# Symb0x76/ChineseChessZero

Measured on NVIDIA B200. Metric: self-play moves/sec at 400 playouts, higher is better.
Workload: dtype bf16

## Files before the change

chinesechesszero_b200/_lib.py:

```python
from __future__ import annotations

import ctypes
import os

import numpy as np
import torch

from . import build as _build

BOARD_BYTES = 96
MAX_MOVES = 128
N_ACTIONS = 2086
PLANE_ELEMS = 10710
KEY_WINDOW = 128

FLAG_CHECK, FLAG_NOMOVES, FLAG_INSUFFICIENT, FLAG_FOURFOLD, FLAG_SIXTY = 1, 2, 4, 8, 16
FLAG_TIE_MASK = FLAG_INSUFFICIENT | FLAG_FOURFOLD | FLAG_SIXTY
STATUS_EXPAND_FAILED, STATUS_TREE_DROPPED = 1, 2
STATUS_NODE_OVERFLOW = STATUS_EXPAND_FAILED
ADVANCE_NEW_GAME, ADVANCE_DROP_TREE, ADVANCE_KEEP = -1, -2, -3
CTL_HEAD, CTL_TAIL, CTL_EXPAND_FAILED, CTL_TREES_DROPPED, CTL_MIN_FREE, CTL_WORDS = 0, 1, 2, 3, 4, 8
NODE_BYTES = 24
MAX_CHILDREN = 119
POLICY_PROBS, POLICY_LOGITS = 0, 1
DEDUP_MAX_BOARDS = 16384
CONV_VARIANT_1CTA, CONV_VARIANT_PAIR, CONV_VARIANT_2PAIRS, CONV_VARIANT_4PAIRS = 1, 2, 2 | 32, 2 | 64

EXPORTS = (
    "ccz_version", "ccz_last_error", "ccz_init", "ccz_action_table", "ccz_set_order_policy", "ccz_get_order_policy",
    "ccz_boards_start",
    "ccz_movegen_encode", "ccz_board_keys_init", "ccz_board_push", "ccz_mcts_pool_init", "ccz_mcts_reset",
    "ccz_mcts_reserve", "ccz_mcts_migrate", "ccz_mcts_select",
    "ccz_mcts_expand_backup", "ccz_mcts_root_visits", "ccz_mcts_advance", "ccz_replay_pack", "ccz_conv3x3_c256", "ccz_conv3x3_plan", "ccz_stem_lookup",
    "ccz_heads_pack", "ccz_conv3x3_c256_count", "ccz_stem_lookup_count", "ccz_heads_pack_rows", "ccz_leaf_unique",
)


class CczError(RuntimeError):
    pass


# ... 334 lines not shown
def conv3x3_c256(x: torch.Tensor, w: torch.Tensor, bias: torch.Tensor, skip: torch.Tensor | None = None,
                 out: torch.Tensor | None = None, variant: int = 0, count: torch.Tensor | None = None) -> torch.Tensor:
    cl = torch.channels_last
    if x.dtype != torch.bfloat16 or w.dtype != torch.bfloat16 or bias.dtype != torch.float32:
        raise CczError("conv3x3_c256: x and w must be bfloat16, bias float32")
    if tuple(x.shape[1:]) != (256, 10, 9) or tuple(w.shape) != (256, 256, 3, 3) or bias.numel() != 256:
        raise CczError("conv3x3_c256: shapes must be x (n,256,10,9), w (256,256,3,3), bias (256,)")
    if not x.is_contiguous(memory_format=cl) or not w.is_contiguous(memory_format=cl):
        raise CczError("conv3x3_c256: x and w must be channels_last")
    if skip is not None and (skip.shape != x.shape or skip.dtype != x.dtype or not skip.is_contiguous(memory_format=cl)):
        raise CczError("conv3x3_c256: skip must match x (bf16, channels_last)")
    if out is None:
        out = torch.empty_like(x, memory_format=cl)
    elif out.shape != x.shape or out.dtype != x.dtype or not out.is_contiguous(memory_format=cl):
        raise CczError("conv3x3_c256: out must match x (bf16, channels_last)")
    if not 0 <= variant < 128:
        raise CczError("conv3x3_c256: variant out of range (see ccz_conv3x3_c256 in include/ccz_b200.h)")
    if not (x.is_cuda and w.is_cuda and bias.is_cuda and out.is_cuda):
        raise CczError("device tensor expected (the C ABI takes device pointers)")
    sk = None if skip is None else skip.data_ptr()
    with torch.cuda.device(x.device):
        if count is None:
            check(load().ccz_conv3x3_c256(x.data_ptr(), w.data_ptr(), bias.data_ptr(), sk, out.data_ptr(), int(x.shape[0]),
                                          int(variant), stream_ptr(x.device)), "ccz_conv3x3_c256")
        else:
            _check_count(count, x.device)
            check(load().ccz_conv3x3_c256_count(x.data_ptr(), w.data_ptr(), bias.data_ptr(), sk, out.data_ptr(), int(x.shape[0]),
                                                count.data_ptr(), int(variant), stream_ptr(x.device)), "ccz_conv3x3_c256_count")
    return out


# ... 60 lines not shown
```

chinesechesszero_b200/csrc/ccz_b200.cu:

```cuda
#include "../../include/ccz_b200.h"

#include <cuda_runtime.h>

#include <cstdio>
#include <cstdlib>
#include <cstring>
#include <utility>
#include <string>

#include "ccz_movegen.cuh"
#include "ccz_mcts.cuh"
#include "ccz_replay.cuh"
#include "ccz_conv.cuh"
#include "ccz_stem.cuh"
#include "ccz_heads.cuh"
#include "ccz_dedup.cuh"

#ifndef CCZ_CONV_DEFAULT_PAIRS
#define CCZ_CONV_DEFAULT_PAIRS 1
#endif

namespace {

thread_local std::string g_err;
// ... 397 lines not shown
    const int threads = 256;
    const long long blocks = (words + threads - 1) / threads;
    if (blocks > 0x7fffffffll) return fail(-1, "ccz_replay_pack: n too large");
    ccz::replay_states_kernel<<<(unsigned)blocks, threads, 0, s>>>(d_hist_boards, d_turn_plane, n,
                                                                   static_cast<uint32_t *>(d_states_f16));
    if (int rc = check_launch("replay_states_kernel")) return rc;
    CCZ_CUDA(cudaMemsetAsync(d_pi, 0, (size_t)2 * n * ccz::N_ACTIONS * sizeof(double), s));
    ccz::replay_pi_kernel<<<(n * 32 + threads - 1) / threads, threads, 0, s>>>(d_acts, d_probs, d_counts, n, d_pi);
    return check_launch("replay_pi_kernel");
}

}

namespace {

int conv3x3_c256_impl(const char *name, const void *d_x, const void *d_w, const float *d_bias, const void *d_skip, void *d_y,
                      int n_boards, const int32_t *d_count, int variant, ccz_stream_t s) {
    namespace cv = ccz::conv;
    std::string e_name(name);
    auto bad = [&](int code, const char *what) { return fail(code, (e_name + ": " + what).c_str()); };
    if (n_boards < 0) return bad(-1, "n_boards < 0");
    if (n_boards == 0) return 0;
    if (!d_x || !d_w || !d_bias || !d_y) return bad(-1, "NULL pointer");
    if (d_y == d_x) return bad(-1, "output must not alias the input (halo reads)");
    if (variant < 0 || variant >= 128) return bad(-1, "bad variant");
    int cta_group = variant & 3;
    const int tail_split = !(variant & 4), dbg = (variant >> 3) & 3;
    int pairs = 1 << ((variant >> 5) & 3);
#ifndef CCZ_CONV_EXPERIMENTS
    if (dbg) return bad(-1, "the load-skipping measurement variants need a -DCCZ_CONV_EXPERIMENTS build");
#endif
    if (variant == 0) { cta_group = 2; pairs = CCZ_CONV_DEFAULT_PAIRS; }
    if (cta_group == 0) cta_group = 2;
    if (cta_group == 3 || pairs > 4 || (cta_group == 1 && pairs != 1))
        return bad(-1, "unsupported variant (cta_group 1|2, pairs 1|2|4, pairs > 1 needs cta_group 2)");
    if (((uintptr_t)d_x | (uintptr_t)d_w | (uintptr_t)d_y | (uintptr_t)d_skip) & 15)
        return bad(-1, "pointers must be 16-byte aligned");
    static cv::Driver drv;
    if (const char *err = cv::driver_init(drv)) return fail(-3, err);
    const long long m = (long long)n_boards * cv::BOARD_HW;
    const int rows_per_tile = cv::BM * cta_group * pairs;
    const int n_tiles = (int)((m + rows_per_tile - 1) / rows_per_tile);
    CUtensorMap tx, tw, ts, ty;
    if (!cv::encode_im2col(drv, &tx, d_x, n_boards)) return bad(-3, "cuTensorMapEncodeIm2col(x) failed");
    if (!cv::encode_rows(drv, &tw, d_w, cv::BN, 9 * cv::C, (uint32_t)(cv::BN / cta_group / pairs)))
        return bad(-3, "cuTensorMapEncodeTiled(w) failed");
    if (!cv::encode_rows(drv, &ty, d_y, (uint64_t)m, cv::C, cv::BM)) return bad(-3, "cuTensorMapEncodeTiled(y) failed");
    if (d_skip) {
        if (!cv::encode_rows(drv, &ts, d_skip, (uint64_t)m, cv::C, cv::BM)) return bad(-3, "cuTensorMapEncodeTiled(skip) failed");
    } else {
        ts = ty;
    }
    cudaError_t e;
#define CCZ_CONV_LAUNCH_C(CG, PAIRS, CNT)                                                                                  \
    (d_skip ? cv::launch_variant<CG, PAIRS, true, CNT>(tx, tw, ts, ty, d_bias, n_tiles, tail_split, dbg, d_count, n_boards, s) \
            : cv::launch_variant<CG, PAIRS, false, CNT>(tx, tw, ts, ty, d_bias, n_tiles, tail_split, dbg, d_count, n_boards, s))
#define CCZ_CONV_LAUNCH(CG, PAIRS) (d_count ? CCZ_CONV_LAUNCH_C(CG, PAIRS, true) : CCZ_CONV_LAUNCH_C(CG, PAIRS, false))
    if (cta_group == 1) e = CCZ_CONV_LAUNCH(1, 1);
    else if (pairs == 1) e = CCZ_CONV_LAUNCH(2, 1);
    else if (pairs == 2) e = CCZ_CONV_LAUNCH(2, 2);
    else e = CCZ_CONV_LAUNCH(2, 4);
#undef CCZ_CONV_LAUNCH
#undef CCZ_CONV_LAUNCH_C
    if (e != cudaSuccess) return fail(-2, "conv3x3_c256_kernel launch", e);
    return 0;
}

int stem_lookup_impl(const char *name, const uint8_t *d_boards, int n, const int32_t *d_count, const void *d_table,
                     const float *d_bias_turn, void *d_y, ccz_stream_t s) {
    namespace st = ccz::stem;
    std::string e_name(name);
    if (n < 0) return fail(-1, (e_name + ": n < 0").c_str());
    if (n == 0) return 0;
    if (!d_boards || !d_table || !d_bias_turn || !d_y) return fail(-1, (e_name + ": NULL pointer").c_str());
    if (((uintptr_t)d_boards & 3) || (((uintptr_t)d_table | (uintptr_t)d_bias_turn | (uintptr_t)d_y) & 15))
        return fail(-1, (e_name + ": pointers must be 16-byte aligned (boards 4-byte)").c_str());
// ... 41 lines not shown
extern "C" {

int ccz_conv3x3_c256(const void *d_x, const void *d_w, const float *d_bias, const void *d_skip, void *d_y, int n_boards,
                     int variant, ccz_stream_t s) {
    return conv3x3_c256_impl("ccz_conv3x3_c256", d_x, d_w, d_bias, d_skip, d_y, n_boards, nullptr, variant, s);
}

int ccz_conv3x3_c256_count(const void *d_x, const void *d_w, const float *d_bias, const void *d_skip, void *d_y, int capacity,
                           const int32_t *d_n_boards, int variant, ccz_stream_t s) {
    if (!d_n_boards) return fail(-1, "ccz_conv3x3_c256_count: d_n_boards is NULL");
    return conv3x3_c256_impl("ccz_conv3x3_c256_count", d_x, d_w, d_bias, d_skip, d_y, capacity, d_n_boards, variant, s);
}

int ccz_conv3x3_plan(int n_boards, int variant, int resident_clusters, int32_t *out) {
    namespace cv = ccz::conv;
    if (n_boards <= 0 || resident_clusters <= 0 || !out || variant < 0 || variant >= 128)
        return fail(-1, "ccz_conv3x3_plan: bad argument");
    int cta_group = variant & 3, pairs = 1 << ((variant >> 5) & 3);
    if (variant == 0) { cta_group = 2; pairs = CCZ_CONV_DEFAULT_PAIRS; }
    if (cta_group == 0) cta_group = 2;
    if (cta_group == 3 || pairs > 4 || (cta_group == 1 && pairs != 1)) return fail(-1, "ccz_conv3x3_plan: unsupported variant");
    const long long m = (long long)n_boards * cv::BOARD_HW;
    const int rows_per_tile = cv::BM * cta_group * pairs;
    const int n_tiles = (int)((m + rows_per_tile - 1) / rows_per_tile);
    const cv::Plan pl = cv::plan_items(n_tiles, resident_clusters, !(variant & 4));
    out[0] = rows_per_tile; out[1] = n_tiles; out[2] = pl.n_items; out[3] = pl.n_full; out[4] = pl.split_log2; out[5] = pl.clusters;
    return 0;
}

int ccz_stem_lookup(const uint8_t *d_boards, int n, const void *d_table, const float *d_bias_turn, void *d_y, ccz_stream_t s) {
    return stem_lookup_impl("ccz_stem_lookup", d_boards, n, nullptr, d_table, d_bias_turn, d_y, s);
}

int ccz_stem_lookup_count(const uint8_t *d_boards, int capacity, const int32_t *d_n_boards, const void *d_table, const float *d_bias_turn,
                          void *d_y, ccz_stream_t s) {
    if (!d_n_boards) return fail(-1, "ccz_stem_lookup_count: d_n_boards is NULL");
    return stem_lookup_impl("ccz_stem_lookup_count", d_boards, capacity, d_n_boards, d_table, d_bias_turn, d_y, s);
}
// ... 36 lines not shown
```

chinesechesszero_b200/csrc/ccz_conv.cuh:

```cuda
#pragma once

#include <cuda.h>
#include <cuda_bf16.h>
#include <cuda_runtime.h>

#include <cstdint>

#ifndef CCZ_CONV_BACKOFF_NS
#define CCZ_CONV_BACKOFF_NS 256
#endif

namespace ccz {
namespace conv {

constexpr int C = 256;
constexpr int BOARD_H = 10, BOARD_W = 9, BOARD_HW = 90;
constexpr int BM = 128;
constexpr int BN = 256;
constexpr int BK = 64;
constexpr int KBLOCKS = 9 * (C / BK);
constexpr int UMMA_K = 16;
constexpr int THREADS = 256;

template <int CG>
struct Cfg {
    static constexpr int B_ROWS = BN / CG;
    static constexpr int A_BYTES = BM * BK * 2;
    static constexpr int B_BYTES = B_ROWS * BK * 2;
    static constexpr int STAGE_BYTES = A_BYTES + B_BYTES;
    static constexpr int STAGES = CG == 2 ? 5 : 3;
    static constexpr int STAGING_BYTES = BM * BN * 2;
    static constexpr int BIAS_BYTES = BN * 4;
    static constexpr int BAR_BYTES = 256;
    static constexpr int SMEM_BYTES = 1024  + STAGES * STAGE_BYTES + STAGING_BYTES + BIAS_BYTES + BAR_BYTES;
};

__device__ __forceinline__ uint32_t smem_u32(const void *p) { return (uint32_t)__cvta_generic_to_shared(p); }

__device__ __forceinline__ uint32_t cluster_ctarank() {
    uint32_t r;
    asm volatile("mov.u32 %0, %%cluster_ctarank;" : "=r"(r));
    return r;
}
__device__ __forceinline__ uint32_t mapa(uint32_t addr, uint32_t rank) {
    uint32_t r;
// ... 172 lines not shown
    asm volatile("barrier.cluster.arrive.release.aligned;\nbarrier.cluster.wait.acquire.aligned;" ::: "memory");
}

__device__ __forceinline__ uint64_t umma_desc_sw128(uint32_t smem_addr) {
    return (uint64_t)((smem_addr >> 4) & 0x3FFF) | (1ull << 16) | (64ull << 32) | (1ull << 46) | (2ull << 61);
}
__host__ __device__ constexpr uint32_t umma_idesc(int m, int n) {
    return (1u << 4) | (1u << 7) | (1u << 10) | ((uint32_t)(n >> 3) << 17) | ((uint32_t)(m >> 4) << 24);
}

__device__ __forceinline__ uint32_t pack_bf16x2(float lo, float hi) {
    __nv_bfloat162 t = __floats2bfloat162_rn(lo, hi);
    return *reinterpret_cast<uint32_t *>(&t);
}

struct WorkItem {
    int tile, n_off, n_w;
};
__device__ __forceinline__ WorkItem work_item(int i, int n_full, int split_log2) {
    if (i < n_full) return {i, 0, BN};
    const int j = i - n_full, n_w = BN >> split_log2;
    return {n_full + (j >> split_log2), (j & ((1 << split_log2) - 1)) * n_w, n_w};
}

struct Plan {
    int n_items, n_full, split_log2, clusters;
};
__host__ __device__ inline Plan plan_items(int n_tiles, int clusters, bool tail_split) {
    const int rem = n_tiles % clusters;
    int split_log2 = 0;
    if (tail_split && rem > 0) {
        while (split_log2 < 2 && (rem << (split_log2 + 1)) <= clusters) ++split_log2;
    }
    Plan p;
    p.split_log2 = split_log2;
    p.n_full = split_log2 ? n_tiles - rem : n_tiles;
    p.n_items = p.n_full + (split_log2 ? rem << split_log2 : 0);
    p.clusters = clusters > p.n_items ? p.n_items : clusters;
    return p;
}

template <int CG, int PAIRS, bool HAS_SKIP, bool DEV_COUNT>
__global__ void __launch_bounds__(THREADS, 1)
conv3x3_c256_kernel(const __grid_constant__ CUtensorMap tm_x, const __grid_constant__ CUtensorMap tm_w,
                    const __grid_constant__ CUtensorMap tm_skip, const __grid_constant__ CUtensorMap tm_y, const float *__restrict__ bias,
                    int n_items, int n_full, int split_log2, int dbg, const int32_t *__restrict__ d_count, int count_cap, int tail_split) {
    using K = Cfg<CG>;
    extern __shared__ uint8_t smem_raw[];
    const uint32_t smem_base = (smem_u32(smem_raw) + 1023u) & ~1023u;
    const uint32_t a_smem = smem_base;
    const uint32_t b_smem = a_smem + K::STAGES * K::A_BYTES;
    const uint32_t staging = b_smem + K::STAGES * K::B_BYTES;
    const uint32_t bias_smem = staging + K::STAGING_BYTES;
    const uint32_t bars = bias_smem + K::BIAS_BYTES;
    const uint32_t bar_full = bars;
    const uint32_t bar_empty = bars + 8 * K::STAGES;
    const uint32_t bar_tfull = bars + 16 * K::STAGES;
    const uint32_t bar_tempty = bar_tfull + 16;
    const uint32_t bar_skip = bar_tempty + 16;
    const uint32_t bar_stfree = bar_skip + 8;
    const uint32_t tmem_slot = bar_stfree + 8;
    uint8_t *const smem_gen = smem_raw + (smem_base - smem_u32(smem_raw));

    const int warp = threadIdx.x >> 5, lane = threadIdx.x & 31;
    static_assert(CG == 2 || PAIRS == 1, "weight multicast needs CTA pairs");
    constexpr int CLUSTER = CG * PAIRS;
    const uint32_t rank = CLUSTER > 1 ? cluster_ctarank() : 0u;
    const uint32_t prank = rank % CG, pair_id = rank / CG, lead_rank = rank - prank;
    const int cluster_id = blockIdx.x / CLUSTER, n_clusters = gridDim.x / CLUSTER;
    if constexpr (DEV_COUNT) {
        const int nb = min(max(*d_count, 0), count_cap), rows_per_tile = BM * CLUSTER;
        const Plan pl = plan_items((nb * BOARD_HW + rows_per_tile - 1) / rows_per_tile, n_clusters, tail_split != 0);
        n_items = pl.n_items;
        n_full = pl.n_full;
        split_log2 = pl.split_log2;
    }

    if (warp == 0 && lane == 0) {
        tma_prefetch_desc(&tm_x);
        tma_prefetch_desc(&tm_w);
        tma_prefetch_desc(&tm_y);
        if (HAS_SKIP) tma_prefetch_desc(&tm_skip);
    }
    if (warp == 1 && lane == 0) {
        for (int i = 0; i < K::STAGES; ++i) {
            mbar_init(bar_full + 8 * i, 1);
            mbar_init(bar_empty + 8 * i, PAIRS);
        }
        for (int i = 0; i < 2; ++i) {
            mbar_init(bar_tfull + 8 * i, 1);
            mbar_init(bar_tempty + 8 * i, 4 * CG);
        }
        mbar_init(bar_skip, 1);
        mbar_init(bar_stfree, 1);
        asm volatile("fence.mbarrier_init.release.cluster;" ::: "memory");
    }
    if (warp == 2) tmem_alloc<CG>(tmem_slot, 512);
    if (warp >= 4) {
        const int t = threadIdx.x - 128;
        reinterpret_cast<float *>(smem_gen + (bias_smem - smem_base))[t] = bias[t];
        reinterpret_cast<float *>(smem_gen + (bias_smem - smem_base))[t + 128] = bias[t + 128];
    }
    tc_fence_before();
    if constexpr (CLUSTER > 1) cluster_sync_all(); else __syncthreads();
    tc_fence_after();
    const uint32_t tmem_base = *reinterpret_cast<volatile uint32_t *>(smem_gen + (tmem_slot - smem_base));

    if (warp == 0) {
        if (lane == 0) {
            const uint32_t full0 = CG == 2 ? mapa(bar_full, lead_rank) : bar_full;
            constexpr int SLICE_ROWS = K::B_ROWS / PAIRS;
            uint16_t mc_mask = 0;
            for (int j = 0; j < PAIRS; ++j) mc_mask |= (uint16_t)(1u << (j * CG + prank));
            int stage = 0;
            uint32_t phase = 0;
            for (int item = cluster_id; item < n_items; item += n_clusters) {
                const WorkItem wi = work_item(item, n_full, split_log2);
                const int m0 = ((wi.tile * PAIRS + (int)pair_id) * CG + (int)prank) * BM;
                const int b_row = wi.n_off + (int)prank * (wi.n_w / CG);
                const int img = m0 / BOARD_HW, rem = m0 - img * BOARD_HW;
                const int p = rem / BOARD_W, q = rem - p * BOARD_W;
                for (int kb = 0; kb < KBLOCKS; ++kb) {
                    const int tap = kb >> 2, c0 = (kb & 3) * BK;
                    const int r = tap / 3, s = tap - 3 * r;
                    mbar_wait(bar_empty + 8 * stage, phase ^ 1);
                    const bool do_a = !((dbg & 2) && (kb & 1)), do_b = !((dbg & 1) && (kb & 1));
                    if (prank == 0) mbar_expect_tx(bar_full + 8 * stage, CG * ((do_a ? K::A_BYTES : 0) + (do_b ? K::B_BYTES : 0)));
                    if (do_a) tma_load_im2col<CG>(a_smem + stage * K::A_BYTES, &tm_x, full0 + 8 * stage, c0, q - 1, p - 1, img, (uint16_t)s, (uint16_t)r);
                    if constexpr (PAIRS == 1) {
                        if (do_b) tma_load_2d<CG>(b_smem + stage * K::B_BYTES, &tm_w, full0 + 8 * stage, kb * BK, b_row);
                    } else {
                        tma_load_2d_mc(b_smem + stage * K::B_BYTES + (int)pair_id * SLICE_ROWS * 128, &tm_w, full0 + 8 * stage, kb * BK,
                                       b_row + (int)pair_id * SLICE_ROWS, mc_mask);
                    }
                    if (++stage == K::STAGES) { stage = 0; phase ^= 1; }
                }
            }
        }
    } else if (warp == 1) {
        if (prank == 0 && lane == 0) {
            constexpr uint16_t mask_cluster = (uint16_t)((1u << CLUSTER) - 1);
            const uint16_t mask_pair = (uint16_t)(((1u << CG) - 1) << lead_rank);
            int stage = 0;
            uint32_t phase = 0, acc = 0, acc_phase = 0;
            for (int item = cluster_id; item < n_items; item += n_clusters) {
                const uint32_t idesc = umma_idesc(BM * CG, work_item(item, n_full, split_log2).n_w);
                mbar_wait_cluster(bar_tempty + 8 * acc, acc_phase ^ 1);
                tc_fence_after();
                const uint32_t d_tmem = tmem_base + acc * BN;
                for (int kb = 0; kb < KBLOCKS; ++kb) {
                    mbar_wait(bar_full + 8 * stage, phase);
                    tc_fence_after();
                    const uint64_t a_desc = umma_desc_sw128(a_smem + stage * K::A_BYTES);
                    const uint64_t b_desc = umma_desc_sw128(b_smem + stage * K::B_BYTES);
#pragma unroll
                    for (int k = 0; k < BK / UMMA_K; ++k)
                        umma_bf16<CG>(d_tmem, a_desc + 2 * k, b_desc + 2 * k, idesc, (uint32_t)((kb | k) != 0));
                    umma_commit<CG>(bar_empty + 8 * stage, mask_cluster);
                    if (++stage == K::STAGES) { stage = 0; phase ^= 1; }
                }
                umma_commit<CG>(bar_tfull + 8 * acc, mask_pair);
                if (++acc == 2) { acc = 0; acc_phase ^= 1; }
            }
        }
    } else if (warp == 3) {
        if (HAS_SKIP && lane == 0) {
            uint32_t it = 0;
            for (int item = cluster_id; item < n_items; item += n_clusters, ++it) {
                const WorkItem wi = work_item(item, n_full, split_log2);
                const int m0 = ((wi.tile * PAIRS + (int)pair_id) * CG + (int)prank) * BM;
                mbar_wait_relaxed(bar_stfree, (it & 1) ^ 1);
                mbar_expect_tx(bar_skip, (wi.n_w / 64) * (BM * 128));
                for (int g = 0; g < wi.n_w / 64; ++g) tma_load_2d<1>(staging + g * (BM * 128), &tm_skip, bar_skip, wi.n_off + g * 64, m0);
            }
        }
    } else if (warp >= 4) {
        const int quarter = warp - 4, row = quarter * 32 + lane;
        const uint32_t tempty0 = CG == 2 ? mapa(bar_tempty, lead_rank) : bar_tempty;
        const float *bias_s = reinterpret_cast<const float *>(smem_gen + (bias_smem - smem_base));
        uint8_t *stg = smem_gen + (staging - smem_base);
        uint32_t acc = 0, acc_phase = 0, it = 0;
        for (int item = cluster_id; item < n_items; item += n_clusters, ++it) {
            const WorkItem wi = work_item(item, n_full, split_log2);
            const int m0 = ((wi.tile * PAIRS + (int)pair_id) * CG + (int)prank) * BM;
            if (HAS_SKIP) mbar_wait_relaxed(bar_skip, it & 1);
            mbar_wait_relaxed(bar_tfull + 8 * acc, acc_phase);
            tc_fence_after();
            const uint32_t t_row = tmem_base + ((uint32_t)(quarter * 32) << 16) + acc * BN;
#pragma unroll 1
            for (int chunk = 0; chunk < wi.n_w / 32; ++chunk) {
                uint32_t v[32];
                tmem_ld32(t_row + chunk * 32, v);
                tmem_ld_wait();
                uint8_t *box_row = stg + (chunk >> 1) * (BM * 128) + row * 128;
#pragma unroll
                for (int j = 0; j < 4; ++j) {
                    const int c16 = (chunk & 1) * 4 + j;
                    uint4 *cell = reinterpret_cast<uint4 *>(box_row + ((c16 ^ (row & 7)) << 4));
                    const float4 b0 = *reinterpret_cast<const float4 *>(bias_s + wi.n_off + chunk * 32 + j * 8);
                    const float4 b1 = *reinterpret_cast<const float4 *>(bias_s + wi.n_off + chunk * 32 + j * 8 + 4);
                    float f[8] = {__uint_as_float(v[j * 8 + 0]) + b0.x, __uint_as_float(v[j * 8 + 1]) + b0.y,
                                  __uint_as_float(v[j * 8 + 2]) + b0.z, __uint_as_float(v[j * 8 + 3]) + b0.w,
                                  __uint_as_float(v[j * 8 + 4]) + b1.x, __uint_as_float(v[j * 8 + 5]) + b1.y,
                                  __uint_as_float(v[j * 8 + 6]) + b1.z, __uint_as_float(v[j * 8 + 7]) + b1.w};
                    if (HAS_SKIP) {
                        const uint4 sk = *cell;
                        const uint32_t w[4] = {sk.x, sk.y, sk.z, sk.w};
#pragma unroll
                        for (int e = 0; e < 4; ++e) {
                            f[2 * e] += __uint_as_float(w[e] << 16);
                            f[2 * e + 1] += __uint_as_float(w[e] & 0xFFFF0000u);
                        }
                    }
                    uint4 o;
                    o.x = pack_bf16x2(fmaxf(f[0], 0.f), fmaxf(f[1], 0.f));
                    o.y = pack_bf16x2(fmaxf(f[2], 0.f), fmaxf(f[3], 0.f));
                    o.z = pack_bf16x2(fmaxf(f[4], 0.f), fmaxf(f[5], 0.f));
                    o.w = pack_bf16x2(fmaxf(f[6], 0.f), fmaxf(f[7], 0.f));
                    *cell = o;
                }
            }
            tc_fence_before();
            __syncwarp();
            if (lane == 0) {
                if constexpr (CG == 2) mbar_arrive_cluster(tempty0 + 8 * acc); else mbar_arrive(bar_tempty + 8 * acc);
            }
            if (++acc == 2) { acc = 0; acc_phase ^= 1; }
            fence_proxy_async();
            asm volatile("bar.sync 1, 128;" ::: "memory");
            if (threadIdx.x == 128) {
                for (int g = 0; g < wi.n_w / 64; ++g) tma_store_2d(&tm_y, staging + g * (BM * 128), wi.n_off + g * 64, m0);
                tma_store_commit();
                tma_store_wait_read();
                if (HAS_SKIP) mbar_arrive(bar_stfree);
            }
            asm volatile("bar.sync 1, 128;" ::: "memory");
        }
        if (threadIdx.x == 128) tma_store_wait_all();
    }

    __syncwarp();
    tc_fence_before();
    if constexpr (CLUSTER > 1) cluster_sync_all(); else __syncthreads();
    if (warp == 2) {
        tc_fence_after();
        tmem_dealloc<CG>(tmem_base, 512);
    }
}

typedef CUresult (*EncodeTiledFn)(CUtensorMap *, CUtensorMapDataType, cuuint32_t, void *, const cuuint64_t *, const cuuint64_t *,
                                  const cuuint32_t *, const cuuint32_t *, CUtensorMapInterleave, CUtensorMapSwizzle, CUtensorMapL2promotion,
// ... 30 lines not shown
    const cuuint32_t es[2] = {1, 1};
    return d.tiled(m, CU_TENSOR_MAP_DATA_TYPE_BFLOAT16, 2, const_cast<void *>(ptr), dims, strides, box, es, CU_TENSOR_MAP_INTERLEAVE_NONE,
                   CU_TENSOR_MAP_SWIZZLE_128B, CU_TENSOR_MAP_L2_PROMOTION_L2_256B, CU_TENSOR_MAP_FLOAT_OOB_FILL_NONE) == CUDA_SUCCESS;
}

inline bool encode_im2col(const Driver &d, CUtensorMap *m, const void *ptr, int n) {
    const cuuint64_t dims[4] = {(cuuint64_t)C, (cuuint64_t)BOARD_W, (cuuint64_t)BOARD_H, (cuuint64_t)n};
    const cuuint64_t strides[3] = {(cuuint64_t)C * 2, (cuuint64_t)C * 2 * BOARD_W, (cuuint64_t)C * 2 * BOARD_HW};
    const int lower[2] = {-1, -1}, upper[2] = {-1, -1};
    const cuuint32_t es[4] = {1, 1, 1, 1};
    return d.im2col(m, CU_TENSOR_MAP_DATA_TYPE_BFLOAT16, 4, const_cast<void *>(ptr), dims, strides, lower, upper, BK, BM, es,
                    CU_TENSOR_MAP_INTERLEAVE_NONE, CU_TENSOR_MAP_SWIZZLE_128B, CU_TENSOR_MAP_L2_PROMOTION_L2_256B,
                    CU_TENSOR_MAP_FLOAT_OOB_FILL_NONE) == CUDA_SUCCESS;
}

template <int CG, int PAIRS, bool HAS_SKIP, bool DEV_COUNT>
inline cudaError_t launch_variant(const CUtensorMap &tx, const CUtensorMap &tw, const CUtensorMap &ts, const CUtensorMap &ty, const float *bias,
                                  int n_tiles, int tail_split, int dbg, const int32_t *d_count, int count_cap, cudaStream_t stream) {
    auto kern = conv3x3_c256_kernel<CG, PAIRS, HAS_SKIP, DEV_COUNT>;
    constexpr int CLUSTER = CG * PAIRS;
    static int max_clusters_dev[64] = {0};
    int dev = 0, n_sm = 0;
    cudaError_t e0 = cudaGetDevice(&dev);
    if (e0 != cudaSuccess) return e0;
    if (dev < 0 || dev >= 64) return cudaErrorInvalidDevice;
    int &max_clusters = max_clusters_dev[dev];
    cudaLaunchConfig_t cfg = {};
    cfg.blockDim = dim3(THREADS);
    cfg.dynamicSmemBytes = Cfg<CG>::SMEM_BYTES;
    cfg.stream = stream;
    cudaLaunchAttribute at[1];
    at[0].id = cudaLaunchAttributeClusterDimension;
    at[0].val.clusterDim.x = CLUSTER;
    at[0].val.clusterDim.y = 1;
    at[0].val.clusterDim.z = 1;
    cfg.attrs = at;
    cfg.numAttrs = 1;
    if (!max_clusters) {
        cudaError_t e = cudaDeviceGetAttribute(&n_sm, cudaDevAttrMultiProcessorCount, dev);
        if (e != cudaSuccess) return e;
        e = cudaFuncSetAttribute(kern, cudaFuncAttributeMaxDynamicSharedMemorySize, Cfg<CG>::SMEM_BYTES);
        if (e != cudaSuccess) return e;
        cfg.gridDim = dim3((unsigned)(n_sm / CLUSTER * CLUSTER));
        int n = 0;
        e = cudaOccupancyMaxActiveClusters(&n, kern, &cfg);
        if (e != cudaSuccess) return e;
        if (n < 1) return cudaErrorInvalidConfiguration;
        max_clusters = n < n_sm / CLUSTER ? n : n_sm / CLUSTER;
    }
    if constexpr (DEV_COUNT) {
        cfg.gridDim = dim3((unsigned)(max_clusters * CLUSTER));
        return cudaLaunchKernelEx(&cfg, kern, tx, tw, ts, ty, bias, 0, 0, 0, dbg, d_count, count_cap, tail_split);
    }
    const Plan pl = plan_items(n_tiles, max_clusters, tail_split != 0);
    cfg.gridDim = dim3((unsigned)(pl.clusters * CLUSTER));
    return cudaLaunchKernelEx(&cfg, kern, tx, tw, ts, ty, bias, pl.n_items, pl.n_full, pl.split_log2, dbg, (const int32_t *)nullptr, 0, 0);
// ... 5 lines not shown
```

Measured before the change: 404.9.

## Add two-M-tile-per-CTA conv variant sharing weight tiles, default for pairs

Adds an MT=2 mode to the 3x3 conv kernel. In this mode each CTA pair computes two 128-row M tiles against one loaded weight (B) stage, which halves B traffic per output row. The mode uses two TMEM accumulators, 8 epilogue warps that split columns, and fewer pipeline stages. It becomes the default when pairs==1, which it is by default. The cost is a larger smem stage, shallower pipelining, more threads, and a more complex MMA and epilogue schedule with new phase-tracking assumptions.

Result: slower. 388.6 (median of 6 runs) (-4.0%).

```diff
diff --git a/chinesechesszero_b200/_lib.py b/chinesechesszero_b200/_lib.py
--- a/chinesechesszero_b200/_lib.py
+++ b/chinesechesszero_b200/_lib.py
@@ -25,6 +25,7 @@
 POLICY_PROBS, POLICY_LOGITS = 0, 1
 DEDUP_MAX_BOARDS = 16384
 CONV_VARIANT_1CTA, CONV_VARIANT_PAIR, CONV_VARIANT_2PAIRS, CONV_VARIANT_4PAIRS = 1, 2, 2 | 32, 2 | 64
+CONV_VARIANT_PAIR_2M = 2 | 128
 
 EXPORTS = (
     "ccz_version", "ccz_last_error", "ccz_init", "ccz_action_table", "ccz_set_order_policy", "ccz_get_order_policy",
@@ -389,7 +390,7 @@
         out = torch.empty_like(x, memory_format=cl)
     elif out.shape != x.shape or out.dtype != x.dtype or not out.is_contiguous(memory_format=cl):
         raise CczError("conv3x3_c256: out must match x (bf16, channels_last)")
-    if not 0 <= variant < 128:
+    if not 0 <= variant < 256:
         raise CczError("conv3x3_c256: variant out of range (see ccz_conv3x3_c256 in include/ccz_b200.h)")
     if not (x.is_cuda and w.is_cuda and bias.is_cuda and out.is_cuda):
         raise CczError("device tensor expected (the C ABI takes device pointers)")
diff --git a/chinesechesszero_b200/csrc/ccz_b200.cu b/chinesechesszero_b200/csrc/ccz_b200.cu
--- a/chinesechesszero_b200/csrc/ccz_b200.cu
+++ b/chinesechesszero_b200/csrc/ccz_b200.cu
@@ -435,6 +435,21 @@
 
 namespace {
 
+struct ConvTiling {
+    int cta_group, pairs, mt;
+};
+const char *conv_tiling(int variant, ConvTiling &t) {
+    if (variant < 0 || variant >= 256) return "bad variant";
+    t.cta_group = variant & 3;
+    t.pairs = 1 << ((variant >> 5) & 3);
+    t.mt = variant & 128 ? 2 : 1;
+    if (variant == 0) { t.cta_group = 2; t.pairs = CCZ_CONV_DEFAULT_PAIRS; t.mt = t.pairs == 1 ? 2 : 1; }
+    if (t.cta_group == 0) t.cta_group = 2;
+    if (t.cta_group == 3 || t.pairs > 4 || (t.cta_group == 1 && t.pairs != 1) || (t.mt == 2 && (t.cta_group != 2 || t.pairs != 1)))
+        return "unsupported variant (cta_group 1|2, pairs 1|2|4, pairs > 1 and two M tiles need cta_group 2, two M tiles need pairs 1)";
+    return nullptr;
+}
+
 int conv3x3_c256_impl(const char *name, const void *d_x, const void *d_w, const float *d_bias, const void *d_skip, void *d_y,
                       int n_boards, const int32_t *d_count, int variant, ccz_stream_t s) {
     namespace cv = ccz::conv;
@@ -444,23 +459,19 @@
     if (n_boards == 0) return 0;
     if (!d_x || !d_w || !d_bias || !d_y) return bad(-1, "NULL pointer");
     if (d_y == d_x) return bad(-1, "output must not alias the input (halo reads)");
-    if (variant < 0 || variant >= 128) return bad(-1, "bad variant");
-    int cta_group = variant & 3;
+    ConvTiling t;
+    if (const char *err = conv_tiling(variant, t)) return bad(-1, err);
+    const int cta_group = t.cta_group, pairs = t.pairs;
     const int tail_split = !(variant & 4), dbg = (variant >> 3) & 3;
-    int pairs = 1 << ((variant >> 5) & 3);
 #ifndef CCZ_CONV_EXPERIMENTS
     if (dbg) return bad(-1, "the load-skipping measurement variants need a -DCCZ_CONV_EXPERIMENTS build");
 #endif
-    if (variant == 0) { cta_group = 2; pairs = CCZ_CONV_DEFAULT_PAIRS; }
-    if (cta_group == 0) cta_group = 2;
-    if (cta_group == 3 || pairs > 4 || (cta_group == 1 && pairs != 1))
-        return bad(-1, "unsupported variant (cta_group 1|2, pairs 1|2|4, pairs > 1 needs cta_group 2)");
     if (((uintptr_t)d_x | (uintptr_t)d_w | (uintptr_t)d_y | (uintptr_t)d_skip) & 15)
         return bad(-1, "pointers must be 16-byte aligned");
     static cv::Driver drv;
     if (const char *err = cv::driver_init(drv)) return fail(-3, err);
     const long long m = (long long)n_boards * cv::BOARD_HW;
-    const int rows_per_tile = cv::BM * cta_group * pairs;
+    const int rows_per_tile = cv::BM * t.mt * cta_group * pairs;
     const int n_tiles = (int)((m + rows_per_tile - 1) / rows_per_tile);
     CUtensorMap tx, tw, ts, ty;
     if (!cv::encode_im2col(drv, &tx, d_x, n_boards)) return bad(-3, "cuTensorMapEncodeIm2col(x) failed");
@@ -473,14 +484,15 @@
         ts = ty;
     }
     cudaError_t e;
-#define CCZ_CONV_LAUNCH_C(CG, PAIRS, CNT)                                                                                  \
-    (d_skip ? cv::launch_variant<CG, PAIRS, true, CNT>(tx, tw, ts, ty, d_bias, n_tiles, tail_split, dbg, d_count, n_boards, s) \
-            : cv::launch_variant<CG, PAIRS, false, CNT>(tx, tw, ts, ty, d_bias, n_tiles, tail_split, dbg, d_count, n_boards, s))
-#define CCZ_CONV_LAUNCH(CG, PAIRS) (d_count ? CCZ_CONV_LAUNCH_C(CG, PAIRS, true) : CCZ_CONV_LAUNCH_C(CG, PAIRS, false))
-    if (cta_group == 1) e = CCZ_CONV_LAUNCH(1, 1);
-    else if (pairs == 1) e = CCZ_CONV_LAUNCH(2, 1);
-    else if (pairs == 2) e = CCZ_CONV_LAUNCH(2, 2);
-    else e = CCZ_CONV_LAUNCH(2, 4);
+#define CCZ_CONV_LAUNCH_C(CG, PAIRS, MT, CNT)                                                                                  \
+    (d_skip ? cv::launch_variant<CG, PAIRS, MT, true, CNT>(tx, tw, ts, ty, d_bias, n_tiles, tail_split, dbg, d_count, n_boards, s) \
+            : cv::launch_variant<CG, PAIRS, MT, false, CNT>(tx, tw, ts, ty, d_bias, n_tiles, tail_split, dbg, d_count, n_boards, s))
+#define CCZ_CONV_LAUNCH(CG, PAIRS, MT) (d_count ? CCZ_CONV_LAUNCH_C(CG, PAIRS, MT, true) : CCZ_CONV_LAUNCH_C(CG, PAIRS, MT, false))
+    if (cta_group == 1) e = CCZ_CONV_LAUNCH(1, 1, 1);
+    else if (t.mt == 2) e = CCZ_CONV_LAUNCH(2, 1, 2);
+    else if (pairs == 1) e = CCZ_CONV_LAUNCH(2, 1, 1);
+    else if (pairs == 2) e = CCZ_CONV_LAUNCH(2, 2, 1);
+    else e = CCZ_CONV_LAUNCH(2, 4, 1);
 #undef CCZ_CONV_LAUNCH
 #undef CCZ_CONV_LAUNCH_C
     if (e != cudaSuccess) return fail(-2, "conv3x3_c256_kernel launch", e);
@@ -552,14 +564,12 @@
 
 int ccz_conv3x3_plan(int n_boards, int variant, int resident_clusters, int32_t *out) {
     namespace cv = ccz::conv;
-    if (n_boards <= 0 || resident_clusters <= 0 || !out || variant < 0 || variant >= 128)
+    ConvTiling t;
+    if (n_boards <= 0 || resident_clusters <= 0 || !out || variant < 0 || variant >= 256)
         return fail(-1, "ccz_conv3x3_plan: bad argument");
-    int cta_group = variant & 3, pairs = 1 << ((variant >> 5) & 3);
-    if (variant == 0) { cta_group = 2; pairs = CCZ_CONV_DEFAULT_PAIRS; }
-    if (cta_group == 0) cta_group = 2;
-    if (cta_group == 3 || pairs > 4 || (cta_group == 1 && pairs != 1)) return fail(-1, "ccz_conv3x3_plan: unsupported variant");
+    if (conv_tiling(variant, t)) return fail(-1, "ccz_conv3x3_plan: unsupported variant");
     const long long m = (long long)n_boards * cv::BOARD_HW;
-    const int rows_per_tile = cv::BM * cta_group * pairs;
+    const int rows_per_tile = cv::BM * t.mt * t.cta_group * t.pairs;
     const int n_tiles = (int)((m + rows_per_tile - 1) / rows_per_tile);
     const cv::Plan pl = cv::plan_items(n_tiles, resident_clusters, !(variant & 4));
     out[0] = rows_per_tile; out[1] = n_tiles; out[2] = pl.n_items; out[3] = pl.n_full; out[4] = pl.split_log2; out[5] = pl.clusters;
diff --git a/chinesechesszero_b200/csrc/ccz_conv.cuh b/chinesechesszero_b200/csrc/ccz_conv.cuh
--- a/chinesechesszero_b200/csrc/ccz_conv.cuh
+++ b/chinesechesszero_b200/csrc/ccz_conv.cuh
@@ -20,15 +20,16 @@
 constexpr int BK = 64;
 constexpr int KBLOCKS = 9 * (C / BK);
 constexpr int UMMA_K = 16;
-constexpr int THREADS = 256;
-
-template <int CG>
+
+template <int CG, int MT>
 struct Cfg {
     static constexpr int B_ROWS = BN / CG;
     static constexpr int A_BYTES = BM * BK * 2;
     static constexpr int B_BYTES = B_ROWS * BK * 2;
-    static constexpr int STAGE_BYTES = A_BYTES + B_BYTES;
-    static constexpr int STAGES = CG == 2 ? 5 : 3;
+    static constexpr int STAGE_BYTES = MT * A_BYTES + B_BYTES;
+    static constexpr int STAGES = MT == 2 ? 3 : CG == 2 ? 5 : 3;
+    static constexpr int EPI_WARPS = 4 * MT;
+    static constexpr int THREADS = 128 + 32 * EPI_WARPS;
     static constexpr int STAGING_BYTES = BM * BN * 2;
     static constexpr int BIAS_BYTES = BN * 4;
     static constexpr int BAR_BYTES = 256;
@@ -231,6 +232,37 @@
     return *reinterpret_cast<uint32_t *>(&t);
 }
 
+template <bool HAS_SKIP>
+__device__ __forceinline__ void epilogue_chunk(const uint32_t (&v)[32], uint8_t *stg, int chunk, int row, const float *bias_c) {
+    uint8_t *box_row = stg + (chunk >> 1) * (BM * 128) + row * 128;
+#pragma unroll
+    for (int j = 0; j < 4; ++j) {
+        const int c16 = (chunk & 1) * 4 + j;
+        uint4 *cell = reinterpret_cast<uint4 *>(box_row + ((c16 ^ (row & 7)) << 4));
+        const float4 b0 = *reinterpret_cast<const float4 *>(bias_c + j * 8);
+        const float4 b1 = *reinterpret_cast<const float4 *>(bias_c + j * 8 + 4);
+        float f[8] = {__uint_as_float(v[j * 8 + 0]) + b0.x, __uint_as_float(v[j * 8 + 1]) + b0.y,
+                      __uint_as_float(v[j * 8 + 2]) + b0.z, __uint_as_float(v[j * 8 + 3]) + b0.w,
+                      __uint_as_float(v[j * 8 + 4]) + b1.x, __uint_as_float(v[j * 8 + 5]) + b1.y,
+                      __uint_as_float(v[j * 8 + 6]) + b1.z, __uint_as_float(v[j * 8 + 7]) + b1.w};
+        if (HAS_SKIP) {
+            const uint4 sk = *cell;
+            const uint32_t w[4] = {sk.x, sk.y, sk.z, sk.w};
+#pragma unroll
+            for (int e = 0; e < 4; ++e) {
+                f[2 * e] += __uint_as_float(w[e] << 16);
+                f[2 * e + 1] += __uint_as_float(w[e] & 0xFFFF0000u);
+            }
+        }
+        uint4 o;
+        o.x = pack_bf16x2(fmaxf(f[0], 0.f), fmaxf(f[1], 0.f));
+        o.y = pack_bf16x2(fmaxf(f[2], 0.f), fmaxf(f[3], 0.f));
+        o.z = pack_bf16x2(fmaxf(f[4], 0.f), fmaxf(f[5], 0.f));
+        o.w = pack_bf16x2(fmaxf(f[6], 0.f), fmaxf(f[7], 0.f));
+        *cell = o;
+    }
+}
+
 struct WorkItem {
     int tile, n_off, n_w;
 };
@@ -257,16 +289,18 @@
     return p;
 }
 
-template <int CG, int PAIRS, bool HAS_SKIP, bool DEV_COUNT>
-__global__ void __launch_bounds__(THREADS, 1)
+template <int CG, int PAIRS, int MT, bool HAS_SKIP, bool DEV_COUNT>
+__global__ void __launch_bounds__(Cfg<CG, MT>::THREADS, 1)
 conv3x3_c256_kernel(const __grid_constant__ CUtensorMap tm_x, const __grid_constant__ CUtensorMap tm_w,
                     const __grid_constant__ CUtensorMap tm_skip, const __grid_constant__ CUtensorMap tm_y, const float *__restrict__ bias,
                     int n_items, int n_full, int split_log2, int dbg, const int32_t *__restrict__ d_count, int count_cap, int tail_split) {
-    using K = Cfg<CG>;
+    using K = Cfg<CG, MT>;
+    static_assert(MT == 1 || (MT == 2 && CG == 2 && PAIRS == 1), "two M tiles per CTA need plain CTA pairs");
+    static_assert(MT == 1 || KBLOCKS % (2 * K::STAGES) == 0, "MT = 2: every tile starts on stage 0 with phase 0");
     extern __shared__ uint8_t smem_raw[];
     const uint32_t smem_base = (smem_u32(smem_raw) + 1023u) & ~1023u;
     const uint32_t a_smem = smem_base;
-    const uint32_t b_smem = a_smem + K::STAGES * K::A_BYTES;
+    const uint32_t b_smem = a_smem + K::STAGES * MT * K::A_BYTES;
     const uint32_t staging = b_smem + K::STAGES * K::B_BYTES;
     const uint32_t bias_smem = staging + K::STAGING_BYTES;
     const uint32_t bars = bias_smem + K::BIAS_BYTES;
@@ -286,7 +320,7 @@
     const uint32_t prank = rank % CG, pair_id = rank / CG, lead_rank = rank - prank;
     const int cluster_id = blockIdx.x / CLUSTER, n_clusters = gridDim.x / CLUSTER;
     if constexpr (DEV_COUNT) {
-        const int nb = min(max(*d_count, 0), count_cap), rows_per_tile = BM * CLUSTER;
+        const int nb = min(max(*d_count, 0), count_cap), rows_per_tile = BM * MT * CLUSTER;
         const Plan pl = plan_items((nb * BOARD_HW + rows_per_tile - 1) / rows_per_tile, n_clusters, tail_split != 0);
         n_items = pl.n_items;
         n_full = pl.n_full;
@@ -306,14 +340,14 @@
         }
         for (int i = 0; i < 2; ++i) {
             mbar_init(bar_tfull + 8 * i, 1);
-            mbar_init(bar_tempty + 8 * i, 4 * CG);
+            mbar_init(bar_tempty + 8 * i, K::EPI_WARPS * CG);
         }
         mbar_init(bar_skip, 1);
         mbar_init(bar_stfree, 1);
         asm volatile("fence.mbarrier_init.release.cluster;" ::: "memory");
     }
     if (warp == 2) tmem_alloc<CG>(tmem_slot, 512);
-    if (warp >= 4) {
+    if (warp >= 4 && warp < 8) {
         const int t = threadIdx.x - 128;
         reinterpret_cast<float *>(smem_gen + (bias_smem - smem_base))[t] = bias[t];
         reinterpret_cast<float *>(smem_gen + (bias_smem - smem_base))[t + 128] = bias[t + 128];
@@ -333,17 +367,29 @@
             uint32_t phase = 0;
             for (int item = cluster_id; item < n_items; item += n_clusters) {
                 const WorkItem wi = work_item(item, n_full, split_log2);
-                const int m0 = ((wi.tile * PAIRS + (int)pair_id) * CG + (int)prank) * BM;
+                const int m0 = ((wi.tile * PAIRS + (int)pair_id) * CG + (int)prank) * BM * MT;
                 const int b_row = wi.n_off + (int)prank * (wi.n_w / CG);
-                const int img = m0 / BOARD_HW, rem = m0 - img * BOARD_HW;
-                const int p = rem / BOARD_W, q = rem - p * BOARD_W;
+                int img[MT], p[MT], q[MT];
+#pragma unroll
+                for (int h = 0; h < MT; ++h) {
+                    const int mh = m0 + h * BM;
+                    img[h] = mh / BOARD_HW;
+                    const int rem = mh - img[h] * BOARD_HW;
+                    p[h] = rem / BOARD_W;
+                    q[h] = rem - p[h] * BOARD_W;
+                }
                 for (int kb = 0; kb < KBLOCKS; ++kb) {
                     const int tap = kb >> 2, c0 = (kb & 3) * BK;
                     const int r = tap / 3, s = tap - 3 * r;
                     mbar_wait(bar_empty + 8 * stage, phase ^ 1);
                     const bool do_a = !((dbg & 2) && (kb & 1)), do_b = !((dbg & 1) && (kb & 1));
-                    if (prank == 0) mbar_expect_tx(bar_full + 8 * stage, CG * ((do_a ? K::A_BYTES : 0) + (do_b ? K::B_BYTES : 0)));
-                    if (do_a) tma_load_im2col<CG>(a_smem + stage * K::A_BYTES, &tm_x, full0 + 8 * stage, c0, q - 1, p - 1, img, (uint16_t)s, (uint16_t)r);
+                    if (prank == 0) mbar_expect_tx(bar_full + 8 * stage, CG * ((do_a ? MT * K::A_BYTES : 0) + (do_b ? K::B_BYTES : 0)));
+                    if (do_a) {
+#pragma unroll
+                        for (int h = 0; h < MT; ++h)
+                            tma_load_im2col<CG>(a_smem + (stage * MT + h) * K::A_BYTES, &tm_x, full0 + 8 * stage, c0, q[h] - 1, p[h] - 1, img[h],
+                                                (uint16_t)s, (uint16_t)r);
+                    }
                     if constexpr (PAIRS == 1) {
                         if (do_b) tma_load_2d<CG>(b_smem + stage * K::B_BYTES, &tm_w, full0 + 8 * stage, kb * BK, b_row);
                     } else {
@@ -358,100 +404,145 @@
         if (prank == 0 && lane == 0) {
             constexpr uint16_t mask_cluster = (uint16_t)((1u << CLUSTER) - 1);
             const uint16_t mask_pair = (uint16_t)(((1u << CG) - 1) << lead_rank);
-            int stage = 0;
-            uint32_t phase = 0, acc = 0, acc_phase = 0;
-            for (int item = cluster_id; item < n_items; item += n_clusters) {
-                const uint32_t idesc = umma_idesc(BM * CG, work_item(item, n_full, split_log2).n_w);
-                mbar_wait_cluster(bar_tempty + 8 * acc, acc_phase ^ 1);
-                tc_fence_after();
-                const uint32_t d_tmem = tmem_base + acc * BN;
-                for (int kb = 0; kb < KBLOCKS; ++kb) {
-                    mbar_wait(bar_full + 8 * stage, phase);
+            if constexpr (MT == 2) {
+                constexpr int S = K::STAGES;
+                auto mma_kb = [&](uint32_t a, int kb, uint32_t idesc) {
+                    const int st = kb % S;
+                    const uint64_t a_desc = umma_desc_sw128(a_smem + (st * MT + (int)a) * K::A_BYTES);
+                    const uint64_t b_desc = umma_desc_sw128(b_smem + st * K::B_BYTES);
+#pragma unroll
+                    for (int k = 0; k < BK / UMMA_K; ++k)
+                        umma_bf16<CG>(tmem_base + a * BN, a_desc + 2 * k, b_desc + 2 * k, idesc, (uint32_t)((kb | k) != 0));
+                };
+                auto wait_full = [&](int kb) {
+                    mbar_wait(bar_full + 8 * (kb % S), (uint32_t)(kb / S) & 1u);
                     tc_fence_after();
-                    const uint64_t a_desc = umma_desc_sw128(a_smem + stage * K::A_BYTES);
-                    const uint64_t b_desc = umma_desc_sw128(b_smem + stage * K::B_BYTES);
-#pragma unroll
-                    for (int k = 0; k < BK / UMMA_K; ++k)
-                        umma_bf16<CG>(d_tmem, a_desc + 2 * k, b_desc + 2 * k, idesc, (uint32_t)((kb | k) != 0));
-                    umma_commit<CG>(bar_empty + 8 * stage, mask_cluster);
-                    if (++stage == K::STAGES) { stage = 0; phase ^= 1; }
+                };
+                uint32_t it = 0;
+                for (int item = cluster_id; item < n_items; item += n_clusters, ++it) {
+                    const uint32_t idesc = umma_idesc(BM * CG, work_item(item, n_full, split_log2).n_w);
+                    mbar_wait_cluster(bar_tempty, (it & 1) ^ 1);
+                    tc_fence_after();
+                    for (int kb = 0; kb < S; ++kb) {
+                        wait_full(kb);
+                        mma_kb(0, kb, idesc);
+                    }
+                    mbar_wait_cluster(bar_tempty + 8, (it & 1) ^ 1);
+                    tc_fence_after();
+                    for (int kb = 0; kb < S; ++kb) {
+                        mma_kb(1, kb, idesc);
+                        umma_commit<CG>(bar_empty + 8 * (kb % S), mask_cluster);
+                    }
+                    for (int kb = S; kb < KBLOCKS - S; ++kb) {
+                        wait_full(kb);
+                        mma_kb(0, kb, idesc);
+                        mma_kb(1, kb, idesc);
+                        umma_commit<CG>(bar_empty + 8 * (kb % S), mask_cluster);
+                    }
+                    for (int kb = KBLOCKS - S; kb < KBLOCKS; ++kb) {
+                        wait_full(kb);
+                        mma_kb(0, kb, idesc);
+                    }
+                    umma_commit<CG>(bar_tfull, mask_pair);
+                    for (int kb = KBLOCKS - S; kb < KBLOCKS; ++kb) {
+                        mma_kb(1, kb, idesc);
+                        umma_commit<CG>(bar_empty + 8 * (kb % S), mask_cluster);
+                    }
+                    umma_commit<CG>(bar_tfull + 8, mask_pair);
                 }
-                umma_commit<CG>(bar_tfull + 8 * acc, mask_pair);
-                if (++acc == 2) { acc = 0; acc_phase ^= 1; }
+            } else {
+                int stage = 0;
+                uint32_t phase = 0, acc = 0, acc_phase = 0;
+                for (int item = cluster_id; item < n_items; item += n_clusters) {
+                    const uint32_t idesc = umma_idesc(BM * CG, work_item(item, n_full, split_log2).n_w);
+                    mbar_wait_cluster(bar_tempty + 8 * acc, acc_phase ^ 1);
+                    tc_fence_after();
+                    const uint32_t d_tmem = tmem_base + acc * BN;
+                    for (int kb = 0; kb < KBLOCKS; ++kb) {
+                        mbar_wait(bar_full + 8 * stage, phase);
+                        tc_fence_after();
+                        const uint64_t a_desc = umma_desc_sw128(a_smem + stage * K::A_BYTES);
+                        const uint64_t b_desc = umma_desc_sw128(b_smem + stage * K::B_BYTES);
+#pragma unroll
+                        for (int k = 0; k < BK / UMMA_K; ++k)
+                            umma_bf16<CG>(d_tmem, a_desc + 2 * k, b_desc + 2 * k, idesc, (uint32_t)((kb | k) != 0));
+                        umma_commit<CG>(bar_empty + 8 * stage, mask_cluster);
+                        if (++stage == K::STAGES) { stage = 0; phase ^= 1; }
+                    }
+                    umma_commit<CG>(bar_tfull + 8 * acc, mask_pair);
+                    if (++acc == 2) { acc = 0; acc_phase ^= 1; }
+                }
             }
         }
     } else if (warp == 3) {
         if (HAS_SKIP && lane == 0) {
-            uint32_t it = 0;
-            for (int item = cluster_id; item < n_items; item += n_clusters, ++it) {
+            uint32_t u = 0;
+            for (int item = cluster_id; item < n_items; item += n_clusters) {
                 const WorkItem wi = work_item(item, n_full, split_log2);
-                const int m0 = ((wi.tile * PAIRS + (int)pair_id) * CG + (int)prank) * BM;
-                mbar_wait_relaxed(bar_stfree, (it & 1) ^ 1);
-                mbar_expect_tx(bar_skip, (wi.n_w / 64) * (BM * 128));
-                for (int g = 0; g < wi.n_w / 64; ++g) tma_load_2d<1>(staging + g * (BM * 128), &tm_skip, bar_skip, wi.n_off + g * 64, m0);
+                const int m0 = ((wi.tile * PAIRS + (int)pair_id) * CG + (int)prank) * BM * MT;
+                for (int h = 0; h < MT; ++h, ++u) {
+                    mbar_wait_relaxed(bar_stfree, (u & 1) ^ 1);
+                    mbar_expect_tx(bar_skip, (wi.n_w / 64) * (BM * 128));
+                    for (int g = 0; g < wi.n_w / 64; ++g)
+                        tma_load_2d<1>(staging + g * (BM * 128), &tm_skip, bar_skip, wi.n_off + g * 64, m0 + h * BM);
+                }
             }
         }
     } else if (warp >= 4) {
-        const int quarter = warp - 4, row = quarter * 32 + lane;
+        const int quarter = warp & 3, col_half = (warp - 4) >> 2, row = quarter * 32 + lane;
         const uint32_t tempty0 = CG == 2 ? mapa(bar_tempty, lead_rank) : bar_tempty;
         const float *bias_s = reinterpret_cast<const float *>(smem_gen + (bias_smem - smem_base));
         uint8_t *stg = smem_gen + (staging - smem_base);
-        uint32_t acc = 0, acc_phase = 0, it = 0;
-        for (int item = cluster_id; item < n_items; item += n_clusters, ++it) {
+        uint32_t u = 0;
+        for (int item = cluster_id; item < n_items; item += n_clusters) {
             const WorkItem wi = work_item(item, n_full, split_log2);
-            const int m0 = ((wi.tile * PAIRS + (int)pair_id) * CG + (int)prank) * BM;
-            if (HAS_SKIP) mbar_wait_relaxed(bar_skip, it & 1);
-            mbar_wait_relaxed(bar_tfull + 8 * acc, acc_phase);
-            tc_fence_after();
-            const uint32_t t_row = tmem_base + ((uint32_t)(quarter * 32) << 16) + acc * BN;
+            for (int h = 0; h < MT; ++h, ++u) {
+                const int m0 = ((wi.tile * PAIRS + (int)pair_id) * CG + (int)prank) * BM * MT + h * BM;
+                const uint32_t acc = u & 1, acc_phase = (u >> 1) & 1;
+                const uint32_t t_row = tmem_base + ((uint32_t)(quarter * 32) << 16) + acc * BN;
+                if constexpr (MT == 1) {
+                    if (HAS_SKIP) mbar_wait_relaxed(bar_skip, u & 1);
+                    mbar_wait_relaxed(bar_tfull + 8 * acc, acc_phase);
+                    tc_fence_after();
 #pragma unroll 1
-            for (int chunk = 0; chunk < wi.n_w / 32; ++chunk) {
-                uint32_t v[32];
-                tmem_ld32(t_row + chunk * 32, v);
-                tmem_ld_wait();
-                uint8_t *box_row = stg + (chunk >> 1) * (BM * 128) + row * 128;
-#pragma unroll
-                for (int j = 0; j < 4; ++j) {
-                    const int c16 = (chunk & 1) * 4 + j;
-                    uint4 *cell = reinterpret_cast<uint4 *>(box_row + ((c16 ^ (row & 7)) << 4));
-                    const float4 b0 = *reinterpret_cast<const float4 *>(bias_s + wi.n_off + chunk * 32 + j * 8);
-                    const float4 b1 = *reinterpret_cast<const float4 *>(bias_s + wi.n_off + chunk * 32 + j * 8 + 4);
-                    float f[8] = {__uint_as_float(v[j * 8 + 0]) + b0.x, __uint_as_float(v[j * 8 + 1]) + b0.y,
-                                  __uint_as_float(v[j * 8 + 2]) + b0.z, __uint_as_float(v[j * 8 + 3]) + b0.w,
-                                  __uint_as_float(v[j * 8 + 4]) + b1.x, __uint_as_float(v[j * 8 + 5]) + b1.y,
-                                  __uint_as_float(v[j * 8 + 6]) + b1.z, __uint_as_float(v[j * 8 + 7]) + b1.w};
-                    if (HAS_SKIP) {
-                        const uint4 sk = *cell;
-                        const uint32_t w[4] = {sk.x, sk.y, sk.z, sk.w};
-#pragma unroll
-                        for (int e = 0; e < 4; ++e) {
-                            f[2 * e] += __uint_as_float(w[e] << 16);
-                            f[2 * e + 1] += __uint_as_float(w[e] & 0xFFFF0000u);
-                        }
-                    }
-                    uint4 o;
-                    o.x = pack_bf16x2(fmaxf(f[0], 0.f), fmaxf(f[1], 0.f));
-                    o.y = pack_bf16x2(fmaxf(f[2], 0.f), fmaxf(f[3], 0.f));
-                    o.z = pack_bf16x2(fmaxf(f[4], 0.f), fmaxf(f[5], 0.f));
-                    o.w = pack_bf16x2(fmaxf(f[6], 0.f), fmaxf(f[7], 0.f));
-                    *cell = o;
+                    for (int chunk = 0; chunk < wi.n_w / 32; ++chunk) {
+                        uint32_t v[32];
+                        tmem_ld32(t_row + chunk * 32, v);
+                        tmem_ld_wait();
+                        epilogue_chunk<HAS_SKIP>(v, stg, chunk, row, bias_s + wi.n_off + chunk * 32);
+                    }
+                    tc_fence_before();
+                    __syncwarp();
+                    if (lane == 0) {
+                        if constexpr (CG == 2) mbar_arrive_cluster(tempty0 + 8 * acc); else mbar_arrive(bar_tempty + 8 * acc);
+                    }
+                } else {
+                    const int nch = wi.n_w / 64;
+                    uint32_t v[4][32];
+                    mbar_wait(bar_tfull + 8 * acc, acc_phase);
+                    tc_fence_after();
+#pragma unroll
+                    for (int c = 0; c < 4; ++c)
+                        if (c < nch) tmem_ld32(t_row + (col_half * nch + c) * 32, v[c]);
+                    tmem_ld_wait();
+                    tc_fence_before();
+                    __syncwarp();
+                    if (lane == 0) mbar_arrive_cluster(tempty0 + 8 * acc);
+                    if (HAS_SKIP) mbar_wait(bar_skip, u & 1);
+#pragma unroll
+                    for (int c = 0; c < 4; ++c)
+                        if (c < nch) epilogue_chunk<HAS_SKIP>(v[c], stg, col_half * nch + c, row, bias_s + wi.n_off + (col_half * nch + c) * 32);
                 }
+                fence_proxy_async();
+                asm volatile("bar.sync 1, %0;" ::"n"(32 * K::EPI_WARPS) : "memory");
+                if (threadIdx.x == 128) {
+                    for (int g = 0; g < wi.n_w / 64; ++g) tma_store_2d(&tm_y, staging + g * (BM * 128), wi.n_off + g * 64, m0);
+                    tma_store_commit();
+                    tma_store_wait_read();
+                    if (HAS_SKIP) mbar_arrive(bar_stfree);
+                }
+                asm volatile("bar.sync 1, %0;" ::"n"(32 * K::EPI_WARPS) : "memory");
             }
-            tc_fence_before();
-            __syncwarp();
-            if (lane == 0) {
-                if constexpr (CG == 2) mbar_arrive_cluster(tempty0 + 8 * acc); else mbar_arrive(bar_tempty + 8 * acc);
-            }
-            if (++acc == 2) { acc = 0; acc_phase ^= 1; }
-            fence_proxy_async();
-            asm volatile("bar.sync 1, 128;" ::: "memory");
-            if (threadIdx.x == 128) {
-                for (int g = 0; g < wi.n_w / 64; ++g) tma_store_2d(&tm_y, staging + g * (BM * 128), wi.n_off + g * 64, m0);
-                tma_store_commit();
-                tma_store_wait_read();
-                if (HAS_SKIP) mbar_arrive(bar_stfree);
-            }
-            asm volatile("bar.sync 1, 128;" ::: "memory");
         }
         if (threadIdx.x == 128) tma_store_wait_all();
     }
@@ -512,10 +603,10 @@
                     CU_TENSOR_MAP_FLOAT_OOB_FILL_NONE) == CUDA_SUCCESS;
 }
 
-template <int CG, int PAIRS, bool HAS_SKIP, bool DEV_COUNT>
+template <int CG, int PAIRS, int MT, bool HAS_SKIP, bool DEV_COUNT>
 inline cudaError_t launch_variant(const CUtensorMap &tx, const CUtensorMap &tw, const CUtensorMap &ts, const CUtensorMap &ty, const float *bias,
                                   int n_tiles, int tail_split, int dbg, const int32_t *d_count, int count_cap, cudaStream_t stream) {
-    auto kern = conv3x3_c256_kernel<CG, PAIRS, HAS_SKIP, DEV_COUNT>;
+    auto kern = conv3x3_c256_kernel<CG, PAIRS, MT, HAS_SKIP, DEV_COUNT>;
     constexpr int CLUSTER = CG * PAIRS;
     static int max_clusters_dev[64] = {0};
     int dev = 0, n_sm = 0;
@@ -524,8 +615,8 @@
     if (dev < 0 || dev >= 64) return cudaErrorInvalidDevice;
     int &max_clusters = max_clusters_dev[dev];
     cudaLaunchConfig_t cfg = {};
-    cfg.blockDim = dim3(THREADS);
-    cfg.dynamicSmemBytes = Cfg<CG>::SMEM_BYTES;
+    cfg.blockDim = dim3(Cfg<CG, MT>::THREADS);
+    cfg.dynamicSmemBytes = Cfg<CG, MT>::SMEM_BYTES;
     cfg.stream = stream;
     cudaLaunchAttribute at[1];
     at[0].id = cudaLaunchAttributeClusterDimension;
@@ -537,7 +628,7 @@
     if (!max_clusters) {
         cudaError_t e = cudaDeviceGetAttribute(&n_sm, cudaDevAttrMultiProcessorCount, dev);
         if (e != cudaSuccess) return e;
-        e = cudaFuncSetAttribute(kern, cudaFuncAttributeMaxDynamicSharedMemorySize, Cfg<CG>::SMEM_BYTES);
+        e = cudaFuncSetAttribute(kern, cudaFuncAttributeMaxDynamicSharedMemorySize, Cfg<CG, MT>::SMEM_BYTES);
         if (e != cudaSuccess) return e;
         cfg.gridDim = dim3((unsigned)(n_sm / CLUSTER * CLUSTER));
         int n = 0;
```
